# darcamo/pyphysim

Measured on AMD Instinct MI355X. Metric: Monte Carlo realizations/sec (whole node) + SER abs-error vs ref, higher is better.
Workload: dtype f64

## Files before the change

pyphysim_amd/csrc/c4_select.hpp:

```cpp
#pragma once
#include <cstdio>
#include "../../include/mcle.h"

namespace mcle {

enum : int { WDEC_GENERIC = 0, WDEC_SLICER = 1, WDEC_QAM_CERT = 2, WDEC_QUAD_CERT = 3, WDEC_AXIS4_CERT = 4 };

enum : int {
    C4_THR_DEFAULT = 0,
    C4_THR_R4_AH4 = 256,
    C4_THR_R16_ALT = 257,
    C4_THR_R16_TABLE = 258,
    C4_THR_R16_FUSED = 259,
    C4_THR_WAVE = 260,
    C4_THR_PLANAR = 261,
    C4_THR_WAVE_ALT = 262,
    C4_THR_PW4 = 263,
    C4_THR_PW4_W2 = 264,
    C4_THR_PW_TIME = 265,
    C4_THR_PW_CLASS = 266,
    C4_THR_PW_PLANES = 267,
    C4_THR_PW_HALVES = 268,
    C4_THR_512 = 512,
    C4_THR_1024 = 1024,
};
constexpr bool c4_threads_accepted(long long v) {
    return v == C4_THR_DEFAULT || (v >= C4_THR_R4_AH4 && v <= C4_THR_PW_HALVES) || v == C4_THR_512 || v == C4_THR_1024;
}

struct C4Query {
    bool f64;
    int fft_size, nt, nr, num_used, cp_size;
    int M;
    int dec;
    long long f64_threads, f64_generic, no_mfma, f32_mfma, mfma_variant;
#ifdef MCLE_EXPERIMENTS
    long long f64_variant;
#endif
};

enum : int { C4_REFUSED_SHAPE = 0, C4_GENERIC, C4_PLANAR, C4_FW, C4_QW, C4_PW, C4_MFMA };

struct C4Plan {
    int family = C4_REFUSED_SHAPE;
    bool f64 = true;
    int n = 0, nt = 0, nr = 0;
    int ah = 0;
    int wps = 0;
    int variant = 0;
    bool td = false, rows = false, halves = false;
    char asked = 0;
    int abl = 0;
};

#ifndef MCLE_PLANAR_F32_WPS_PLUS
#define MCLE_PLANAR_F32_WPS_PLUS 2
#endif
#ifndef MCLE_PLANAR_F64_256_WPS3
#define MCLE_PLANAR_F64_256_WPS3 0
#endif
constexpr int planar_wps(bool f64, int n, int nt, int nr, int w64) {
    if (!f64 && w64 <= 3 && ((n == 256 && !(nt == 4 && nr == 4)) || (n == 512 && nr == 2))) return w64 + MCLE_PLANAR_F32_WPS_PLUS;
    if (MCLE_PLANAR_F64_256_WPS3 && f64 && n == 256 && nr <= 3 && w64 == 2) return 3;
    return w64;
}

constexpr int planar_r4_ah(int nr) { return nr == 3 ? 3 : 2; }
constexpr int planar_r4_wps(bool f64, int n, int nt, int nr) {
    const int w64 = nr == 3 ? 2 : nr == 2 ? (n == 256 ? 2 : n == 2048 ? 4 : 3) : (n <= 512 ? 3 : 4);
    return planar_wps(f64, n, nt, nr, w64);
}

#ifdef MCLE_EXPERIMENTS
constexpr bool c4_abl_wave(long long v) { return (v >= 32 && v <= 1024 && (v & (v - 1)) == 0) || v == 2016; }
constexpr bool c4_abl_qw(long long v) { return c4_abl_wave(v) || v == 384; }
constexpr bool c4_abl_planar(long long v) { return c4_abl_qw(v) || v == 1920; }
#endif

inline bool c4_select_planar(const C4Query& q, C4Plan& p) {
    const int n = q.fft_size, nt = q.nt, nr = q.nr;
    const long long thr = q.f64_threads;
    if (!(n == 256 || n == 512 || n == 1024 || n == 2048) || nr < 2 || nr > 4 || nt < 1 || nt > nr) return false;
    if (n == 256 && nt == 2 && nr == 2) return false;
    p.family = C4_PLANAR;
    p.ah = planar_r4_ah(nr);
    p.wps = planar_r4_wps(q.f64, n, nt, nr);
    p.variant = 0;
    if (n == 1024 && nr == 4) {
        const int r16_wps = q.f64 ? 2 : 4, r16_var = q.f64 ? 12 : 4;
        if (nt < 4) {
            if (thr == C4_THR_DEFAULT) p.ah = 4, p.wps = r16_wps, p.variant = r16_var;
            return true;
        }
#ifdef MCLE_EXPERIMENTS
        if (q.f64 && q.f64_variant >= 1 && q.f64_variant <= 3) {
            p.variant = (int)q.f64_variant;
            return true;
        }
        if (q.f64 && c4_abl_planar(q.f64_variant)) {
            p.ah = 4, p.wps = 2, p.variant = 12 | (int)q.f64_variant;
            return true;
        }
#endif
        if (thr == C4_THR_512) return true;
        p.ah = 4, p.wps = r16_wps, p.variant = r16_var;
        if (thr == C4_THR_R4_AH4) p.wps = 2, p.variant = 0;
        else if (q.f64 && thr == C4_THR_R16_TABLE) p.variant = 28;
        else if (q.f64 && thr == C4_THR_R16_ALT) p.variant = 4;
        else if (!q.f64 && thr == C4_THR_R16_ALT) p.wps = 3;
        else if (!q.f64 && thr == C4_THR_R16_FUSED) p.variant = 12;
        return true;
    }
    if (n == 2048 && nr == 4 && (thr == C4_THR_512 || (thr != C4_THR_1024 && (nt == 4 || !q.f64)))) p.ah = 4, p.wps = 2;
    return true;
}

inline C4Plan c4_select(const C4Query& q) {
    const int n = q.fft_size, nt = q.nt, nr = q.nr;
    const long long thr = q.f64_threads;
    const bool sq4 = nt == 4 && nr == 4;
    C4Plan p;
    p.f64 = q.f64, p.n = n, p.nt = nt, p.nr = nr;
    if (!q.f64 && q.f32_mfma && !q.no_mfma && n == 1024 && sq4) {
        p.family = C4_MFMA;
        p.variant = q.mfma_variant ? (int)q.mfma_variant : 36;
        return p;
    }
    const bool has_generic = nt == nr && (nt == 2 || nt == 4);
    const bool want_generic = has_generic && (q.f64_generic || (!q.f64 && q.no_mfma));
    if (!want_generic) {
        const bool wave = q.num_used == n && (q.cp_size & 1) == 0 && q.M <= 256 && q.dec != WDEC_GENERIC;
        const bool wave_thr = thr == C4_THR_DEFAULT || thr == C4_THR_WAVE || thr == C4_THR_WAVE_ALT;
        if (wave && n == 256 && has_generic && wave_thr) {
            p.family = C4_FW;
            p.wps = (thr == C4_THR_WAVE_ALT) == q.f64 ? 2 : 3;
#ifdef MCLE_EXPERIMENTS
            if (q.f64 && sq4 && c4_abl_wave(q.f64_variant)) p.wps = 3, p.abl = (int)q.f64_variant;
#endif
            return p;
        }
        const bool pw_thr = thr == C4_THR_DEFAULT || (thr >= C4_THR_PW_TIME && thr <= C4_THR_PW_HALVES) ||
                            (n == 1024 ? thr == C4_THR_PW4 || thr == C4_THR_PW4_W2 : thr == C4_THR_WAVE || thr == C4_THR_WAVE_ALT);
        if (wave && q.f64 && sq4 && (n == 512 || n == 1024 || n == 2048) && pw_thr) {
            p.family = C4_PW;
            p.wps = n == 2048 ? 2 : 3;
            p.td = thr == C4_THR_PW_TIME;
            p.rows = !p.td && thr != C4_THR_PW_CLASS;
            p.halves = p.rows && (thr == C4_THR_PW_HALVES || (thr != C4_THR_PW_PLANES && n != 512));
            p.asked = thr == C4_THR_PW_PLANES ? 'x' : thr == C4_THR_PW_HALVES ? 'h' : 0;
            if (n != 2048) {
                if (thr == C4_THR_WAVE_ALT || thr == C4_THR_PW4_W2) p.wps = 2;
#ifdef MCLE_EXPERIMENTS
                if ((thr < C4_THR_PW_CLASS || thr > C4_THR_PW_HALVES) && c4_abl_wave(q.f64_variant))
                    p.wps = 3, p.halves = false, p.abl = (int)q.f64_variant;
#endif
            }
            return p;
        }
        if (wave && q.f64 && sq4 && n == 1024 && wave_thr && (q.dec == WDEC_SLICER || q.dec == WDEC_QAM_CERT || q.dec == WDEC_QUAD_CERT)) {
            p.family = C4_QW;
            p.wps = thr == C4_THR_WAVE_ALT ? 2 : 3;
#ifdef MCLE_EXPERIMENTS
            if (c4_abl_qw(q.f64_variant)) p.wps = 3, p.abl = (int)q.f64_variant;
#endif
            return p;
        }
        if (c4_select_planar(q, p)) return p;
    }
    if (has_generic) p.family = C4_GENERIC;
    return p;
}

inline void c4_plan_tag(const C4Plan& p, char* out, int len) {
    const char* dt = p.f64 ? "f64" : "f32";
    switch (p.family) {
        case C4_GENERIC: std::snprintf(out, (size_t)len, "mimo_ofdm_generic<%d,%d> %s", p.n, p.nt, dt); break;
        case C4_PLANAR: std::snprintf(out, (size_t)len, "mimo_ofdm_planar<%d,%d,%d> %s ah%d w%d v%d", p.n, p.nt, p.nr, dt, p.ah, p.wps, p.variant); break;
        case C4_FW: std::snprintf(out, (size_t)len, "mimo_ofdm_fw<%d> %s w%d", p.nt, dt, p.wps); break;
        case C4_QW: std::snprintf(out, (size_t)len, "mimo_ofdm_qw w%d", p.wps); break;
        case C4_PW:
            std::snprintf(out, (size_t)len, "mimo_ofdm_pw<%d>/%s%s%s", p.n / 256, p.td ? "time" : "freq", p.wps == (p.n == 2048 ? 2 : 3) ? "" : "/w2",
                          !p.td && !p.rows ? "/a" : p.asked == 'x' ? "/x" : p.asked == 'h' ? "/h" : "");
            break;
        case C4_MFMA: std::snprintf(out, (size_t)len, "mimo_ofdm_mfma v%d", p.variant); break;
        default: if (len > 0) out[0] = 0; break;
    }
}

}
```

pyphysim_amd/csrc/mimo_planar_common.hpp:

```cpp
#pragma once
#include <type_traits>
#include <utility>

#include "fft.hpp"
#include "fft_r16.hpp"
#include "mimo.hpp"
#include "modem.hpp"
#include "philox.hpp"
#include "totals.hpp"
#include "pipe_common.hpp"

namespace mcle {

struct MimoParams {
    int cp, num_used, n_ofdm_sym;
    int mmse;
    double noise_var;
};

template <int NT, int NR> constexpr int d64_rec() { return 2 * NT * NR + 1; }


template <typename T, int N, int NT, int NR>
__global__ __launch_bounds__(64) void k_mimo_filters_planar(MimoParams pp, uint64_t seed, uint64_t first, uint64_t count,
                                                            cx<T>* __restrict__ recs) {
    constexpr int kRec = d64_rec<NT, NR>();
    const uint64_t rl = (uint64_t)blockIdx.x * 64 + threadIdx.x;
    if (rl >= count) return;
    const double rx_scale = sqrt((double)(pp.num_used + pp.cp)) / (double)N;
    const Rng rng(seed, first + rl);
    cx<T>* rec = recs + rl * kRec;
    double2 H[NR][NT], G[NT][NR];
#pragma unroll
    for (int r = 0; r < NR; ++r)
#pragma unroll
        for (int a = 0; a < NT; ++a) {
            const cx<T> h = cn_sample<T>(rng, STREAM_CHAN, (uint64_t)(r * NT + a), (T)1);
            rec[r * NT + a] = h;
            H[r][a] = mk<double>((double)h.x, (double)h.y);
        }
    const bool ok = blast_filter<NT, NR>(H, pp.mmse ? pp.noise_var : 0.0, G);
#pragma unroll
    for (int a = 0; a < NT; ++a)
#pragma unroll
        for (int r = 0; r < NR; ++r) rec[NT * NR + a * NR + r] = mk<T>((T)(G[a][r].x * rx_scale), (T)(G[a][r].y * rx_scale));
    rec[2 * NT * NR] = mk<T>(ok ? (T)0 : (T)1, (T)0);
}

template <typename T, int N, int NT, int NR, typename Link>
inline int launch_sliced_planar(mcle_ctx* ctx, const MimoParams& pp, uint64_t seed, uint64_t first, uint64_t count, uint64_t k_slice,
                                uint32_t* d_sym, uint32_t* d_bit, Link&& link) {
    return launch_sliced(ctx, first, count, k_slice, d64_rec<NT, NR>() * sizeof(cx<T>), d_sym, d_bit,
                         [&](void* recs, uint64_t at, uint64_t n) {
                             hipLaunchKernelGGL((k_mimo_filters_planar<T, N, NT, NR>), dim3((unsigned)((n + 63) / 64)), dim3(64), 0,
                                                ctx->stream, pp, seed, at, n, (cx<T>*)recs);
                         },
                         link);
}

__device__ __forceinline__ void swap32_pair(double a, double b, double& x, double& y) {
    const auto lo = __builtin_amdgcn_permlane32_swap((unsigned)__double2loint(a), (unsigned)__double2loint(b), false, false);
    const auto hi = __builtin_amdgcn_permlane32_swap((unsigned)__double2hiint(a), (unsigned)__double2hiint(b), false, false);
    x = __hiloint2double((int)hi[0], (int)lo[0]);
    y = __hiloint2double((int)hi[1], (int)lo[1]);
}
__device__ __forceinline__ void swap32_pair(float a, float b, float& x, float& y) {
    const auto v = __builtin_amdgcn_permlane32_swap(__float_as_uint(a), __float_as_uint(b), false, false);
    x = __uint_as_float(v[0]);
    y = __uint_as_float(v[1]);
}

__device__ __forceinline__ double2 cn_words(uint32_t x0, uint32_t x1, double sigma, const double* s_bm) {
    return cn_from_words_lds(x0, x1, sigma, s_bm);
}
__device__ __forceinline__ float2 cn_words(uint32_t x0, uint32_t x1, float sigma, const double*) { return cn_from_words(x0, x1, sigma); }

}
```

pyphysim_amd/csrc/pipeline_mimo_pw.hip:

```cpp
#include "mimo_planar_common.hpp"
#include "walk_f64.hpp"

namespace mcle {

constexpr int kPwPlane = 4 * 272;
__host__ __device__ __forceinline__ int pw_slot(int a, int e) { return a * 272 + e + (e >> 4); }
__host__ __device__ __forceinline__ int pw_mtime(int h, int c) { return (c & 3) * 64 + (c >> 2) * 16 + (h & 3) * 4 + (h >> 2); }
template <int NW> constexpr int pw_lab_stride() { return 16 * NW + 16; }
template <int NW> constexpr size_t pw_static_lds() {
    return (size_t)((kBmLdsDoubles + 1) & ~1) * sizeof(double) + (size_t)64 * pw_lab_stride<NW>() + 2 * (d64_rec<4, 4>() + 1) * sizeof(double2) +
           64 * sizeof(unsigned) + sizeof(WgTotals);
}

__device__ __forceinline__ void pw_row_swap(uint32_t& x, uint32_t& y) {
#if defined(__HIP_DEVICE_COMPILE__)
#if __has_builtin(__builtin_amdgcn_permlane16_swap)
    const auto s = __builtin_amdgcn_permlane16_swap(x, y, false, false);
    x = s[0];
    y = s[1];
#else
    const bool odd = (__lane_id() & 16) != 0;
    const uint32_t give = odd ? x : y, got = (uint32_t)__shfl_xor((int)give, 16);
    if (odd) x = got;
    else y = got;
#endif
#endif
}

template <int NW, int J, bool STUB>
__device__ __forceinline__ void pw_first_stage(const unsigned char* lab_row, const double2* s_txtab, const double2* __restrict__ g_tw,
                                               double2 (&v)[16]) {
    const uint4* lab = reinterpret_cast<const uint4*>(lab_row);
    if constexpr (NW == 4) {
#pragma unroll
        for (int i = 0; i < 4; ++i) {
            const uint4 L = lab[i];
            const uint32_t wds[4] = {L.x, L.y, L.z, L.w};
#pragma unroll
            for (int uu = 0; uu < 4; ++uu) {
                const int u = 4 * i + uu;
                const uint32_t w = wds[uu];
                double2 X0, X1, X2, X3;
                if constexpr (STUB) {
                    X0 = X1 = X2 = X3 = mk<double>((double)w, 1.0);
                } else {
                    X0 = s_txtab[w & 0xFFu];
                    X1 = s_txtab[(w >> 8) & 0xFFu];
                    X2 = s_txtab[(w >> 16) & 0xFFu];
                    X3 = s_txtab[w >> 24];
                }
                const double2 A = (J & 1) ? csub(X0, X2) : cadd(X0, X2);
                const double2 B = (J & 1) ? csub(X1, X3) : cadd(X1, X3);
                double2 S;
                if constexpr (J == 0) S = cadd(A, B);
                else if constexpr (J == 1) S = mk<double>(A.x - B.y, A.y + B.x);
                else if constexpr (J == 2) S = csub(A, B);
                else S = mk<double>(A.x + B.y, A.y - B.x);
                if constexpr (J == 0) v[u] = S;
                else if (u == 0) v[u] = S;
                else v[u] = cmulc(S, g_tw[16 * J * u]);
            }
        }
    } else if constexpr (NW == 8) {
        constexpr double kH = 0.70710678118654752440;
// ... 16 lines not shown
#pragma unroll
                    for (int q = 0; q < 8; ++q) X[q] = mk<double>((double)(w0 + w1), 1.0);
                } else {
#pragma unroll
                    for (int q = 0; q < 4; ++q) {
                        X[q] = s_txtab[(w0 >> (8 * q)) & 0xFFu];
                        X[q + 4] = s_txtab[(w1 >> (8 * q)) & 0xFFu];
                    }
                }
                double2 A[4];
#pragma unroll
                for (int q = 0; q < 4; ++q) A[q] = (J & 1) ? csub(X[q], X[q + 4]) : cadd(X[q], X[q + 4]);
                const double2 B0 = cadd(A[0], rotJ(A[2])), B1 = cadd(A[1], rotJ(A[3]));
                double2 S;
                if constexpr (J == 0) S = cadd(B0, B1);
                else if constexpr (J == 2) S = mk<double>(B0.x - B1.y, B0.y + B1.x);
                else if constexpr (J == 4) S = csub(B0, B1);
                else if constexpr (J == 6) S = mk<double>(B0.x + B1.y, B0.y - B1.x);
                else {
                    constexpr double c = (J == 1 || J == 7) ? kH : -kH, sn = (J == 1 || J == 3) ? kH : -kH;
                    S = mk<double>(B0.x + (c * B1.x - sn * B1.y), B0.y + (sn * B1.x + c * B1.y));
                }
                if constexpr (J == 0) v[u] = S;
                else if (u == 0) v[u] = S;
                else v[u] = cmulc(S, g_tw[16 * J * u]);
            }
        }
    } else {
        static_assert(NW == 2, "first stage");
#pragma unroll
        for (int i = 0; i < 2; ++i) {
            const uint4 L = lab[i];
            const uint32_t wds[4] = {L.x, L.y, L.z, L.w};
#pragma unroll
            for (int uu = 0; uu < 8; ++uu) {
                const int u = 8 * i + uu;
                const uint32_t w = wds[uu >> 1] >> (16 * (uu & 1));
                double2 X0, X1;
                if constexpr (STUB) {
                    X0 = X1 = mk<double>((double)(w & 0xFFFFu), 1.0);
                } else {
                    X0 = s_txtab[w & 0xFFu];
                    X1 = s_txtab[(w >> 8) & 0xFFu];
                }
                const double2 S = J ? csub(X0, X1) : cadd(X0, X1);
                if constexpr (J == 0) v[u] = S;
                else if (u == 0) v[u] = S;
                else v[u] = cmulc(S, g_tw[16 * J * u]);
            }
        }
    }
}

template <int NW, int DEC, int WPS, bool TD = false, int ABL = 0, bool ROWS = !TD, bool XCH = ROWS && !TD>
__global__ __launch_bounds__(64 * NW, WPS) void k_run_mimo_ofdm_pw(MimoParams pp, ModemParams<double> mp, uint64_t seed, uint64_t first,
                                                                   uint64_t count, const double2* __restrict__ g_tw,
                                                                   const double2* __restrict__ g_recs, mcle_counters* counters,
                                                                   uint32_t* __restrict__ sym_out, uint32_t* __restrict__ bit_out) {
    using T = double;
    constexpr int N = 256 * NW, NT = 4, NR = 4, kRec = d64_rec<NT, NR>(), TB = 64 * NW, UU = 16 / NW;
    constexpr int kLabStride = pw_lab_stride<NW>();
    static_assert(NW == 2 || NW == 4 || NW == 8, "wavefronts per realization");
    static_assert(!(TD && ROWS), "the time-domain form keeps the map wavefront = class");
    static_assert(!XCH || (ROWS && ABL == 0), "the exchange in complex halves belongs to the default form by lane row");
    constexpr bool kAhead = ROWS && ABL == 0;
#ifdef MCLE_PW_LATE_B5
    constexpr bool kLateB5 = XCH && kAhead;
#else
    constexpr bool kLateB5 = false;
#endif
    constexpr int kLogNW = NW == 2 ? 1 : NW == 4 ? 2 : 3;
    extern __shared__ __attribute__((aligned(16))) char pw_smem[];
    constexpr int kBm = (kBmLdsDoubles + 1) & ~1;
    __shared__ __attribute__((aligned(16))) double s_bm[kBm];
    __shared__ __attribute__((aligned(16))) unsigned char s_lab[64 * kLabStride];
    __shared__ __attribute__((aligned(16))) cx<T> s_rec[2 * (kRec + 1)];
    __shared__ unsigned s_part[64];
    __shared__ WgTotals totals;
    static_assert(sizeof(s_bm) + sizeof(s_lab) + sizeof(s_rec) + sizeof(s_part) + sizeof(totals) == pw_static_lds<NW>(), "launcher's LDS sum");
    T* s_R = reinterpret_cast<T*>(pw_smem);
    cx<T>* s_table = reinterpret_cast<cx<T>*>(s_R + NW * kPwPlane);
    cx<T>* s_txtab = s_table + ((mp.M + 1) & ~1);

    const int tid = threadIdx.x, lane = tid & 63;
    const int j = __builtin_amdgcn_readfirstlane(tid >> 6);
    const int pj = j & 1;
    const int cp = pp.cp;
    const int per_sym = N * NT;
    const uint64_t row = (uint64_t)pp.n_ofdm_sym * (N + cp);
    const T sigma = (T)sqrt(pp.noise_var);
    const T tx_scale = (T)(1.0 / sqrt((double)NT) / sqrt((double)(N + cp)));
    const T tab_scale = TD ? tx_scale : tx_scale * (T)N;
    const uint32_t mask = (uint32_t)(mp.M - 1);
    for (int m = tid; m < mp.M; m += TB) {
        const cx<T> c = mp.g_table[m];
        s_table[m] = c;
        s_txtab[m] = cscale(c, tab_scale);
    }
    if constexpr (ROWS) bm_tables_to_lds_pairs(s_bm, tid, TB);
    else bm_tables_to_lds(s_bm, tid, TB);
    if (tid == 0) wg_zero(totals);

    T* s_mine = s_R + j * kPwPlane;
    uint2* s_words_mine = reinterpret_cast<uint2*>(s_mine);
    using Pass = std::conditional_t<kAhead, uint32_t, uint64_t>;
    Pass it = 0;
    uint64_t rl_prev = 0;
    cx<T> rec_next = mk<T>(0, 0);
    if (tid < kRec && blockIdx.x < count) rec_next = g_recs[(uint64_t)blockIdx.x * kRec + tid];
    unsigned step = 0;
    if constexpr (kAhead) {
        step = gridDim.x;
        asm volatile("" : "+s"(step));
    }
    auto grid_step = [&]() -> unsigned {
        if constexpr (kAhead) return step;
        else return gridDim.x;
    };
    __syncthreads();
    for (uint64_t rl = blockIdx.x; rl < count; rl += grid_step(), ++it) {
        const Rng rng(seed, first + rl);
        const int buf = (int)(it & 1);
        if (tid < kRec) {
            s_rec[buf * (kRec + 1) + tid] = rec_next;
            if (rl + grid_step() < count) rec_next = g_recs[(rl + grid_step()) * kRec + tid];
        }
        const cx<T>* s_H = s_rec + buf * (kRec + 1);
        const cx<T>* s_G = s_H + NT * NR;
        unsigned se = 0, be = 0;
        for (int os = 0; os < pp.n_ofdm_sym; ++os) {
            if constexpr (!kLateB5) {
                if (it > 0 || os > 0) __syncthreads();
            }
            if constexpr (ROWS && !(ABL & 128)) __builtin_amdgcn_s_waitcnt(0xC07F);
            {
                const int t = opaque(tid);
                Words4 dw;
                if constexpr (ABL & 32) dw.w[0] = dw.w[1] = dw.w[2] = dw.w[3] = (uint32_t)t * 0x01010101u;
                else dw = rng.block(STREAM_DATA, (uint32_t)(((uint64_t)os * per_sym) >> 4) + (uint32_t)t);
                const int q = (t >> 6) ^ (NW / 2), u = (t & 63) >> 2;
#pragma unroll
                for (int s = 0; s < 4; ++s) {
                    const uint32_t w = dw.w[s] & (mask * 0x01010101u);
                    const int g = 4 * (t & 3) + s;
                    unsigned char* dst = s_lab + g * kLabStride + NW * u + q;
#pragma unroll
                    for (int a = 0; a < 4; ++a) dst[a * 16 * kLabStride] = (unsigned char)(w >> (8 * a));
                }
            }
            if constexpr (!ROWS) {
                const int ln = opaque(lane);
                const int r = ln >> 4, h = ln & 15;
                const uint64_t i00 = (uint64_t)r * row + (uint64_t)os * (N + cp) + cp + (j & ~1) + 32 * NW * pj + NW * (uint64_t)pw_mtime(h, 0);
                const uint32_t b0 = (uint32_t)(i00 >> 1);
                uint2* w_even = reinterpret_cast<uint2*>(s_R + (j & ~1) * kPwPlane) + (8 * pj) * 64 + ln;
                uint2* w_odd = reinterpret_cast<uint2*>(s_R + (j | 1) * kPwPlane) + (8 * pj) * 64 + ln;
#pragma unroll
                for (int cc = 0; cc < 8; ++cc) {
                    Words4 b;
                    if constexpr (ABL & 128) b.w[0] = b.w[1] = b.w[2] = b.w[3] = b0 + cc;
                    else b = rng.block(STREAM_NOISE, b0 + (uint32_t)(NW / 2) * (uint32_t)pw_mtime(0, cc));
                    w_even[cc * 64] = make_uint2(b.w[0], b.w[1]);
                    w_odd[cc * 64] = make_uint2(b.w[2], b.w[3]);
                }
            }
            auto account_prev = [&]() {
                if (tid == 0 && os == 0 && it > 0) {
                    const unsigned* qq = s_part + (buf ^ 1) * 32;
                    unsigned ts = 0, tb = 0;
#pragma unroll
                    for (int i = 0; i < NW; ++i) {
                        ts += qq[2 * i];
                        tb += qq[2 * i + 1];
                    }
                    uint64_t rp = rl_prev;
                    if constexpr (kAhead) {
                        uint64_t here = rl;
                        asm volatile("" : "+s"(here));
                        rp = here - step;
                    }
                    wg_account(totals, ts, tb, s_rec[(buf ^ 1) * (kRec + 1) + 2 * NT * NR].x != 0.0, rp, sym_out, bit_out);
                }
            };
            if constexpr (!ROWS) {
                __syncthreads();
                account_prev();
            }
            cx<T> v[16];
            if constexpr (TD) {
                const int ln = opaque(lane);
                const unsigned char* lab = s_lab + ln * kLabStride;
                if constexpr (NW == 4) {
                    switch (j) {
                        case 0: pw_first_stage<4, 0, (ABL & 32) != 0>(lab, s_txtab, g_tw, v); break;
                        case 1: pw_first_stage<4, 1, (ABL & 32) != 0>(lab, s_txtab, g_tw, v); break;
                        case 2: pw_first_stage<4, 2, (ABL & 32) != 0>(lab, s_txtab, g_tw, v); break;
                        default: pw_first_stage<4, 3, (ABL & 32) != 0>(lab, s_txtab, g_tw, v); break;
                    }
                } else if constexpr (NW == 8) {
                    switch (j) {
                        case 0: pw_first_stage<8, 0, (ABL & 32) != 0>(lab, s_txtab, g_tw, v); break;
                        case 1: pw_first_stage<8, 1, (ABL & 32) != 0>(lab, s_txtab, g_tw, v); break;
                        case 2: pw_first_stage<8, 2, (ABL & 32) != 0>(lab, s_txtab, g_tw, v); break;
                        case 3: pw_first_stage<8, 3, (ABL & 32) != 0>(lab, s_txtab, g_tw, v); break;
                        case 4: pw_first_stage<8, 4, (ABL & 32) != 0>(lab, s_txtab, g_tw, v); break;
                        case 5: pw_first_stage<8, 5, (ABL & 32) != 0>(lab, s_txtab, g_tw, v); break;
                        case 6: pw_first_stage<8, 6, (ABL & 32) != 0>(lab, s_txtab, g_tw, v); break;
                        default: pw_first_stage<8, 7, (ABL & 32) != 0>(lab, s_txtab, g_tw, v); break;
                    }
                } else {
                    if (j == 0) pw_first_stage<2, 0, (ABL & 32) != 0>(lab, s_txtab, g_tw, v);
                    else pw_first_stage<2, 1, (ABL & 32) != 0>(lab, s_txtab, g_tw, v);
                }
            }
            if constexpr (TD && !(ABL & 64)) {
                const int g = opaque(lane) & 15;
                R16Tw64<T> tw;
#pragma unroll
                for (int m = 1; m <= 3; ++m) {
                    tw.a1[m - 1] = g_tw[g * (NW * m + j)];
                    tw.a2[m - 1] = g_tw[4 * NW * g * m];
                }
                const cx<T> f0 = g_tw[g * j];
                r16_pass<T, true, false, 0, false, true, true>(nullptr, nullptr, 0, tw, nullptr, 0, v, v);
#pragma unroll
                for (int q = 0; q < 4; ++q) v[q] = cmulc(v[q], f0);
            }
            uint2 nw[16];
            if constexpr (!ROWS) {
                const int ln = opaque(lane);
#pragma unroll
                for (int c = 0; c < 16; ++c) nw[c] = s_words_mine[c * 64 + ln];
            }
            if constexpr (TD) {
                const int ln = opaque(lane);
                const int a = ln >> 4, g = ln & 15;
// ... 98 lines not shown
                const int wbase = pw_slot(a, g), rbase = pw_slot(a, 16 * g);
                T xr[16];
                if constexpr (kLateB5) {
#pragma unroll
                    for (int c = 0; c < 16; ++c) asm volatile("" : "+v"(v[c].x), "+v"(v[c].y));
                    if (it > 0 || os > 0) __syncthreads();
                }
#pragma unroll
                for (int c = 0; c < 16; ++c) s_mine[rbase + c] = v[c].x;
                walk_wave_order();
#pragma unroll
                for (int u = 0; u < 16; ++u) xr[u] = s_mine[wbase + 17 * u];
                walk_wave_order();
#pragma unroll
                for (int c = 0; c < 16; ++c) s_mine[rbase + c] = v[c].y;
                walk_wave_order();
#pragma unroll
                for (int u = 0; u < 16; ++u) v[u] = mk<T>(xr[u], s_mine[wbase + 17 * u]);
            }
            if constexpr (!(ABL & 512)) {
                if constexpr (!kAhead) {
                    const int g = opaque(lane) & 15;
#pragma unroll
                    for (int m = 1; m <= 3; ++m) {
                        tw1.a1[m - 1] = g_tw[NW * g * m];
                        tw1.a2[m - 1] = g_tw[4 * NW * g * m];
                    }
                }
                r16_pass<T, false, true, 0, false, true, true>(nullptr, nullptr, 0, tw1, nullptr, 0, v, v);
            }
            T er[NW][UU], ei[NW][UU];
            cx<T> ez[NW][UU];
            constexpr uint32_t kTwBytes = (uint32_t)sizeof(cx<T>);
            uint32_t kp0 = 0;
            static_assert(16 * kTwBytes * (NW - 1) * (UU - 1) < 4096, "the load's immediate offset");
            auto tw_at = [&](int m, int uu) {
                const char* lane_base = reinterpret_cast<const char*>(g_tw) + (size_t)(kTwBytes * (uint32_t)m * kp0);
                return *reinterpret_cast<const cx<T>*>(lane_base + 16 * (int)kTwBytes * m * uu);
            };
            cx<T> twb[2][NW - 1];
            uint4 lab_ahead = make_uint4(0, 0, 0, 0);
            cx<T> hA_ahead = mk<T>(0, 0), gA_ahead = mk<T>(0, 0);
            if constexpr (XCH) {
                const int ln = opaque(lane);
                const int r = ln >> 4, g = ln & 15;
                constexpr int UH = UU / 2, kSl = 272 / 2;
                cx<T>* s_X = reinterpret_cast<cx<T>*>(s_R);
                const int wA = (4 * j + r) * kSl + g;
                const int rA = NW * r * kSl + g + 16 * UH * j;
                const int rB = NW == 2 ? (4 * (r & 1) + j) * kSl + g + 16 * UH * (r >> 1) : j * kSl + g + 16 * UH * (NW / 4) * r;
                r16_wave_sync();
#pragma unroll
                for (int u = 0; u < 16; ++u) asm volatile("" : "+v"(v[u].x));
                account_prev();
#pragma unroll
                for (int u = 0; u < 16; ++u) asm volatile("" : "+v"(v[u].y));
#pragma unroll
                for (int jw = 0; jw < NW; ++jw)
#pragma unroll
                    for (int uu = 0; uu < UH; ++uu) s_X[wA + 16 * (UH * jw + uu)] = v[UU * jw + uu];
                __syncthreads();
#pragma unroll
                for (int jj = 0; jj < NW; ++jj)
#pragma unroll
                    for (int uu = 0; uu < UH; ++uu) ez[jj][uu] = s_X[rA + jj * kSl + 16 * uu];
#pragma unroll
                for (int jw = 0; jw < NW; ++jw)
#pragma unroll
                    for (int uu = UH; uu < UU; ++uu) s_X[rA + jw * kSl + 16 * (uu - UH)] = v[UU * jw + uu];
                kp0 = (uint32_t)opaque((ln & 15) + 16 * UU * j);
#pragma unroll
                for (int m = 1; m < NW; ++m) twb[0][m - 1] = tw_at(m, 0);
                lab_ahead = *reinterpret_cast<const uint4*>(s_lab + ln * kLabStride + 16 * j);
                hA_ahead = s_H[(ln & 3) * NT + (ln >> 4)];
                gA_ahead = s_G[(ln & 3) * NR + (ln >> 4)];
                __syncthreads();
#pragma unroll
                for (int jj = 0; jj < NW; ++jj) {
                    const int off = NW == 2 ? 2 * jj * kSl : (jj & 3) * NW * kSl + 16 * UH * (jj >> 2);
#pragma unroll
                    for (int uu = UH; uu < UU; ++uu) ez[jj][uu] = s_X[rB + off + 16 * (uu - UH)];
                }
            } else {
                const int ln = opaque(lane);
                const int r = ln >> 4, g = ln & 15;
                constexpr int kClass = ROWS ? 272 : kPwPlane;
                const int wpos = r * 272 + g + (ROWS ? 16 * (((4 * j + r) >> kLogNW) & 1) : 0);
                const int rpos = (ROWS ? NW * r * 272 + 16 * (r & 1) : r * 272) + g + 16 * UU * j;
                r16_wave_sync();
#pragma unroll
                for (int u = 0; u < 16; ++u) s_mine[wpos + 16 * u] = v[u].x;
                __syncthreads();
                if constexpr (ROWS) account_prev();
#pragma unroll
                for (int jj = 0; jj < NW; ++jj)
#pragma unroll
                    for (int uu = 0; uu < UU; ++uu) er[jj][uu] = s_R[jj * kClass + rpos + 16 * uu];
                __syncthreads();
#pragma unroll
                for (int u = 0; u < 16; ++u) s_mine[wpos + 16 * u] = v[u].y;
                if constexpr (kAhead) {
                    kp0 = (uint32_t)opaque((ln & 15) + 16 * UU * j);
#pragma unroll
                    for (int m = 1; m < NW; ++m) twb[0][m - 1] = tw_at(m, 0);
                    lab_ahead = *reinterpret_cast<const uint4*>(s_lab + ln * kLabStride + 16 * j);
                    hA_ahead = s_H[(ln & 3) * NT + (ln >> 4)];
                    gA_ahead = s_G[(ln & 3) * NR + (ln >> 4)];
                }
                __syncthreads();
#pragma unroll
                for (int jj = 0; jj < NW; ++jj)
#pragma unroll
                    for (int uu = 0; uu < UU; ++uu) ei[jj][uu] = s_R[jj * kClass + rpos + 16 * uu];
            }
            if constexpr (!(ABL & 1024)) {
                const int ln = opaque(lane);
                if constexpr (!kAhead) kp0 = (uint32_t)opaque((ln & 15) + 16 * UU * j);
                auto ex = [&](int jj, int uu) {
                    if constexpr (XCH) return ez[jj][uu];
                    else return mk<T>(er[jj][uu], ei[jj][uu]);
                };
                auto tw_of = [&](int m, int uu) {
                    if constexpr (kAhead) return twb[uu & 1][m - 1];
                    else return tw_at(m, uu);
                };
#pragma unroll
                for (int uu = 0; uu < UU; ++uu) {
                    if constexpr (kAhead) {
                        if (uu + 1 < UU) {
#pragma unroll
                            for (int m = 1; m < NW; ++m) twb[(uu + 1) & 1][m - 1] = tw_at(m, uu + 1);
                        }
                        __builtin_amdgcn_sched_barrier(0);
                    }
                    if constexpr (NW == 4) {
                        const cx<T> w1 = tw_of(1, uu), w2 = tw_of(2, uu), w3 = tw_of(3, uu);
                        const cx<T> u0 = ex(0, uu);
                        const cx<T> u1 = cmul(ex(1, uu), w1);
                        const cx<T> u2 = cmul(ex(2, uu), w2);
                        const cx<T> u3 = cmul(ex(3, uu), w3);
                        CxOps<T>::template bfly4<false>(u0, u1, u2, u3, v[4 * uu], v[4 * uu + 1], v[4 * uu + 2], v[4 * uu + 3]);
                    } else if constexpr (NW == 8) {
                        cx<T> x[8];
                        x[0] = ex(0, uu);
#pragma unroll
                        for (int jj = 1; jj < 8; ++jj) x[jj] = cmul(ex(jj, uu), tw_of(jj, uu));
// ... 44 lines not shown
                            yi[jj] = __builtin_amdgcn_mfma_f64_4x4x4f64(him, X[jj].x, v[4 * i + jj].y, 0, 0, 0);
                        }
#pragma unroll
                        for (int jj = 0; jj < 4; ++jj) {
                            yr[jj] = __builtin_amdgcn_mfma_f64_4x4x4f64(nhim, X[jj].y, yr[jj], 0, 0, 0);
                            yi[jj] = __builtin_amdgcn_mfma_f64_4x4x4f64(hre, X[jj].y, yi[jj], 0, 0, 0);
                            v[4 * i + jj] = mk<T>(yr[jj], yi[jj]);
                        }
                    }
                }
                if constexpr (!(ABL & 1024)) {
                cx<T> gA;
                if constexpr (kAhead) gA = gA_ahead;
                else gA = s_G[(ln & 3) * NR + (ln >> 4)];
                const T gre = gA.x, gim = gA.y, ngim = -gA.y;
#pragma unroll
                for (int i = 0; i < 4; ++i) {
                    cx<T> e[4];
#pragma unroll
                    for (int jj = 0; jj < 4; ++jj) {
                        const int u = 4 * i + jj;
                        T xr = __builtin_amdgcn_mfma_f64_4x4x4f64(gre, v[u].x, 0.0, 0, 0, 0);
                        T xi = __builtin_amdgcn_mfma_f64_4x4x4f64(gim, v[u].x, 0.0, 0, 0, 0);
                        xr = __builtin_amdgcn_mfma_f64_4x4x4f64(ngim, v[u].y, xr, 0, 0, 0);
                        xi = __builtin_amdgcn_mfma_f64_4x4x4f64(gre, v[u].y, xi, 0, 0, 0);
                        e[jj] = mk<T>(xr, xi);
                    }
                    if constexpr (DEC == WDEC_SLICER || DEC == WDEC_QAM_CERT) {
                        walk_qam_count4<DEC == WDEC_QAM_CERT>(mp, s_table, e, wds[i], se, be);
                    } else {
                        int tx[4];
#pragma unroll
                        for (int jj = 0; jj < 4; ++jj) tx[jj] = (int)((wds[i] >> (8 * jj)) & 0xFFu);
                        walk_decide<DEC, 4>(mp, s_table, nullptr, e, tx, se, be);
                    }
                }
                } else {
                    T keep = er[0][0] + ei[NW - 1][UU - 1];
                    if constexpr (!TD) {
#pragma unroll
                        for (int u = 0; u < 16; ++u) keep += v[u].x + v[u].y;
                    }
                    se += (unsigned)(keep == 0.5) + (wds[0] == 0x12345u);
                }
            }
        }
        if constexpr (kAhead) {
            se = walk_wave_total(se);
            be = walk_wave_total(be);
        } else {
            se = wave_sum_u32(se);
            be = wave_sum_u32(be);
        }
        if (lane == 0) {
            s_part[buf * 32 + 2 * j] = se;
            s_part[buf * 32 + 2 * j + 1] = be;
        }
        rl_prev = rl;
    }
    __syncthreads();
    if (tid == 0) {
        if (it > 0) {
            const int buf = (int)((it - 1) & 1);
            const unsigned* qq = s_part + buf * 32;
            unsigned ts = 0, tb = 0;
#pragma unroll
            for (int i = 0; i < NW; ++i) {
                ts += qq[2 * i];
                tb += qq[2 * i + 1];
            }
            if constexpr (kAhead) rl_prev = blockIdx.x + (uint64_t)(it - 1) * step;
            wg_account(totals, ts, tb, s_rec[buf * (kRec + 1) + 2 * NT * NR].x != 0.0, rl_prev, sym_out, bit_out);
        }
        wg_flush(totals, counters, (unsigned long long)per_sym * pp.n_ofdm_sym, (unsigned long long)per_sym * pp.n_ofdm_sym * mp.bits);
    }
}

template <int NW, int WPS, bool TD, int ABL, bool ROWS, bool XCH>
static int launch_mimo_ofdm_pw(mcle_ctx* ctx, const C4Plan& plan, const mcle_mimo_ofdm_cfg* cfg, uint64_t seed, uint64_t first,
                               uint64_t count, mcle_counters* d_counters, uint32_t* d_sym, uint32_t* d_bit) {
    using T = double;
    constexpr int N = 256 * NW, NT = 4, NR = 4;
    int rc;
    void* tw = nullptr;
    if ((rc = ctx->get_twiddles(N, MCLE_F64, &tw))) return rc;
    MimoParams pp{cfg->cp_size, cfg->num_used, cfg->n_ofdm_sym, cfg->mmse, cfg->noise_var};
    ModemParams<T> mp = pipe_modem<T>(ctx, cfg->demod_method);
    const int dec = walk_dec_kind(ctx, mp);
    mp.grid.G = 0;
    const size_t tab_len = ((size_t)mp.M + 1) & ~(size_t)1;
    const size_t dyn = (size_t)NW * kPwPlane * sizeof(T) + 2 * tab_len * sizeof(cx<T>);
    const size_t lds = dyn + pw_static_lds<NW>();
    MCLE_REQUIRE(lds + 512 <= (size_t)160 * 1024, "part-wave MIMO-OFDM kernel: %zu B of LDS do not fit", lds);
    auto kern = k_run_mimo_ofdm_pw<NW, WDEC_SLICER, WPS, TD, ABL, ROWS, XCH>;
    switch (dec) {
        case WDEC_QAM_CERT: kern = k_run_mimo_ofdm_pw<NW, WDEC_QAM_CERT, WPS, TD, ABL, ROWS, XCH>; break;
        case WDEC_QUAD_CERT: kern = k_run_mimo_ofdm_pw<NW, WDEC_QUAD_CERT, WPS, TD, ABL, ROWS, XCH>; break;
        case WDEC_AXIS4_CERT: kern = k_run_mimo_ofdm_pw<NW, WDEC_AXIS4_CERT, WPS, TD, ABL, ROWS, XCH>; break;
        default: break;
    }
    MCLE_HIP(hipFuncSetAttribute((const void*)kern, hipFuncAttributeMaxDynamicSharedMemorySize, (int)dyn));
    int per_cu = (int)((size_t)160 * 1024 / (lds + 512));
    if (per_cu < 1) per_cu = 1;
    const int by_waves = WPS * 4 / NW;
    if (per_cu > by_waves) per_cu = by_waves;
    const uint64_t resident = (uint64_t)ctx->n_cu * per_cu;
    static_assert(XCH ? ROWS && ABL == 0 : true, "the exchange in complex halves: default form by lane row only");
    set_c4_kernel(ctx, plan);
    const uint64_t kSlice = 1ull << 20;
    return launch_sliced_planar<T, N, NT, NR>(ctx, pp, seed, first, count, kSlice, d_sym, d_bit,
                                              [&](void* recs, uint64_t at, uint64_t n, uint32_t* sym, uint32_t* bit) {
        const unsigned grid = (unsigned)oversubscribed_grid(ctx, resident, n, 8, NW == 4 ? 32 : 16);
        hipLaunchKernelGGL(kern, dim3(grid), dim3(64 * NW), dyn, ctx->stream, pp, mp, seed, at, n, (const cx<T>*)tw, (const cx<T>*)recs,
                           d_counters, sym, bit);
    });
}

int launch_mimo_ofdm_pw(mcle_ctx* ctx, const C4Plan& p, const mcle_mimo_ofdm_cfg* cfg, uint64_t seed, uint64_t first, uint64_t count,
                        mcle_counters* d_counters, uint32_t* d_sym, uint32_t* d_bit) {
#define MCLE_PW(NW_, WPS_, TD_, ABL_, ROWS_, XCH_)                                                                              \
    if (p.n == 256 * NW_ && p.wps == WPS_ && p.td == TD_ && p.abl == ABL_ && p.rows == ROWS_ && p.halves == XCH_)               \
        return launch_mimo_ofdm_pw<NW_, WPS_, TD_, ABL_, ROWS_, XCH_>(ctx, p, cfg, seed, first, count, d_counters, d_sym, d_bit);
#define MCLE_PW_SIZE(NW_, WPS_)                                                                                                 \
    MCLE_PW(NW_, WPS_, false, 0, false, false) MCLE_PW(NW_, WPS_, false, 0, true, true) MCLE_PW(NW_, WPS_, false, 0, true, false) \
    MCLE_PW(NW_, WPS_, true, 0, false, false)
    MCLE_PW_SIZE(2, 3) MCLE_PW(2, 2, false, 0, true, false)
    MCLE_PW_SIZE(4, 3) MCLE_PW(4, 2, false, 0, true, true)
    MCLE_PW_SIZE(8, 2)
#ifdef MCLE_EXPERIMENTS
#define MCLE_PW_ABL(V_)                                                                                                         \
    MCLE_PW(2, 3, true, V_, false, false) MCLE_PW(2, 3, false, V_, true, false) MCLE_PW(4, 3, true, V_, false, false)           \
    MCLE_PW(4, 3, false, V_, true, false)
    MCLE_PW_ABL(32) MCLE_PW_ABL(64) MCLE_PW_ABL(128) MCLE_PW_ABL(256) MCLE_PW_ABL(512) MCLE_PW_ABL(1024) MCLE_PW_ABL(2016)
#undef MCLE_PW_ABL
#endif
#undef MCLE_PW_SIZE
#undef MCLE_PW
    MCLE_REQUIRE(false, "internal: no part-wave MIMO-OFDM kernel <%d> w%d time %d rows %d halves %d ablation %d", p.n / 256, p.wps, (int)p.td,
                 (int)p.rows, (int)p.halves, p.abl);
}

}
```

Baseline: 50.41 million.

## Move part-wave per-realization error accounting into a separate fold kernel

```diff
diff --git a/pyphysim_amd/csrc/c4_select.hpp b/pyphysim_amd/csrc/c4_select.hpp
--- a/pyphysim_amd/csrc/c4_select.hpp
+++ b/pyphysim_amd/csrc/c4_select.hpp
@@ -21,11 +21,13 @@
     C4_THR_PW_CLASS = 266,
     C4_THR_PW_PLANES = 267,
     C4_THR_PW_HALVES = 268,
+    C4_THR_PW_INLOOP = 269,
+    C4_THR_PW_FOLD = 270,
     C4_THR_512 = 512,
     C4_THR_1024 = 1024,
 };
 constexpr bool c4_threads_accepted(long long v) {
-    return v == C4_THR_DEFAULT || (v >= C4_THR_R4_AH4 && v <= C4_THR_PW_HALVES) || v == C4_THR_512 || v == C4_THR_1024;
+    return v == C4_THR_DEFAULT || (v >= C4_THR_R4_AH4 && v <= C4_THR_PW_FOLD) || v == C4_THR_512 || v == C4_THR_1024;
 }
 
 struct C4Query {
@@ -50,6 +52,7 @@
     int variant = 0;
     bool td = false, rows = false, halves = false;
     char asked = 0;
+    bool fold = false;
     int abl = 0;
 };
 
@@ -70,6 +73,8 @@
     const int w64 = nr == 3 ? 2 : nr == 2 ? (n == 256 ? 2 : n == 2048 ? 4 : 3) : (n <= 512 ? 3 : 4);
     return planar_wps(f64, n, nt, nr, w64);
 }
+
+constexpr bool c4_pw_fold_default(int n) { return n == 512 || n == 2048; }
 
 #ifdef MCLE_EXPERIMENTS
 constexpr bool c4_abl_wave(long long v) { return (v >= 32 && v <= 1024 && (v & (v - 1)) == 0) || v == 2016; }
@@ -139,7 +144,7 @@
 #endif
             return p;
         }
-        const bool pw_thr = thr == C4_THR_DEFAULT || (thr >= C4_THR_PW_TIME && thr <= C4_THR_PW_HALVES) ||
+        const bool pw_thr = thr == C4_THR_DEFAULT || (thr >= C4_THR_PW_TIME && thr <= C4_THR_PW_FOLD) ||
                             (n == 1024 ? thr == C4_THR_PW4 || thr == C4_THR_PW4_W2 : thr == C4_THR_WAVE || thr == C4_THR_WAVE_ALT);
         if (wave && q.f64 && sq4 && (n == 512 || n == 1024 || n == 2048) && pw_thr) {
             p.family = C4_PW;
@@ -147,14 +152,15 @@
             p.td = thr == C4_THR_PW_TIME;
             p.rows = !p.td && thr != C4_THR_PW_CLASS;
             p.halves = p.rows && (thr == C4_THR_PW_HALVES || (thr != C4_THR_PW_PLANES && n != 512));
-            p.asked = thr == C4_THR_PW_PLANES ? 'x' : thr == C4_THR_PW_HALVES ? 'h' : 0;
+            p.asked = thr == C4_THR_PW_PLANES ? 'x' : thr == C4_THR_PW_HALVES ? 'h' : thr == C4_THR_PW_INLOOP ? 'k' : thr == C4_THR_PW_FOLD ? 'f' : 0;
             if (n != 2048) {
                 if (thr == C4_THR_WAVE_ALT || thr == C4_THR_PW4_W2) p.wps = 2;
 #ifdef MCLE_EXPERIMENTS
-                if ((thr < C4_THR_PW_CLASS || thr > C4_THR_PW_HALVES) && c4_abl_wave(q.f64_variant))
+                if ((thr < C4_THR_PW_CLASS || thr > C4_THR_PW_FOLD) && c4_abl_wave(q.f64_variant))
                     p.wps = 3, p.halves = false, p.abl = (int)q.f64_variant;
 #endif
             }
+            p.fold = p.rows && p.abl == 0 && p.wps == (n == 2048 ? 2 : 3) && (p.asked == 'f' || (p.asked == 0 && c4_pw_fold_default(n)));
             return p;
         }
         if (wave && q.f64 && sq4 && n == 1024 && wave_thr && (q.dec == WDEC_SLICER || q.dec == WDEC_QAM_CERT || q.dec == WDEC_QUAD_CERT)) {
@@ -180,7 +186,7 @@
         case C4_QW: std::snprintf(out, (size_t)len, "mimo_ofdm_qw w%d", p.wps); break;
         case C4_PW:
             std::snprintf(out, (size_t)len, "mimo_ofdm_pw<%d>/%s%s%s", p.n / 256, p.td ? "time" : "freq", p.wps == (p.n == 2048 ? 2 : 3) ? "" : "/w2",
-                          !p.td && !p.rows ? "/a" : p.asked == 'x' ? "/x" : p.asked == 'h' ? "/h" : "");
+                          !p.td && !p.rows ? "/a" : p.asked == 'x' ? "/x" : p.asked == 'h' ? "/h" : p.asked == 'k' ? "/k" : p.asked == 'f' ? "/f" : "");
             break;
         case C4_MFMA: std::snprintf(out, (size_t)len, "mimo_ofdm_mfma v%d", p.variant); break;
         default: if (len > 0) out[0] = 0; break;
diff --git a/pyphysim_amd/csrc/fold_counts.hpp b/pyphysim_amd/csrc/fold_counts.hpp
--- /dev/null
+++ b/pyphysim_amd/csrc/fold_counts.hpp
@@ -0,0 +1,74 @@
+#pragma once
+#include "totals.hpp"
+
+namespace mcle {
+
+constexpr int kFoldThreads = 1024;
+
+template <int NW>
+__global__ __launch_bounds__(kFoldThreads) void k_fold_counts(const uint2* __restrict__ part, const double2* __restrict__ recs,
+                                                              int rec_stride, int flag_at, uint64_t n, mcle_counters* counters,
+                                                              uint32_t* __restrict__ sym_out, uint32_t* __restrict__ bit_out,
+                                                              unsigned long long n_sym, unsigned long long n_bits) {
+    static_assert(NW == 2 || NW == 4 || NW == 8, "pairs per realization: 16-byte reads");
+    __shared__ unsigned long long s_tot[kFoldThreads / 64][6];
+    const int tid = threadIdx.x, lane = tid & 63, wave = tid >> 6;
+    unsigned long long t[6] = {0ull, 0ull, 0ull, 0ull, 0ull, 0ull};
+    const uint64_t stride = (uint64_t)gridDim.x * kFoldThreads;
+    for (uint64_t rl = (uint64_t)blockIdx.x * kFoldThreads + tid; rl < n; rl += stride) {
+        const uint4* q = reinterpret_cast<const uint4*>(part + rl * NW);
+        unsigned se = 0, be = 0;
+#pragma unroll
+        for (int i = 0; i < NW / 2; ++i) {
+            const uint4 w = q[i];
+            se += w.x + w.z;
+            be += w.y + w.w;
+        }
+        const bool skipped = recs[rl * (uint64_t)rec_stride + (uint64_t)flag_at].x != 0.0;
+        if (sym_out) sym_out[rl] = skipped ? 0xFFFFFFFFu : se;
+        if (bit_out) bit_out[rl] = skipped ? 0xFFFFFFFFu : be;
+        if (skipped) {
+            ++t[5];
+        } else {
+            ++t[4];
+            t[0] += se;
+            t[1] += (unsigned long long)se * se;
+            t[2] += be;
+            t[3] += (unsigned long long)be * be;
+        }
+    }
+#pragma unroll
+    for (int k = 0; k < 6; ++k) {
+#pragma unroll
+        for (int d = 32; d >= 1; d >>= 1) t[k] += __shfl_down(t[k], d, 64);
+        if (lane == 0) s_tot[wave][k] = t[k];
+    }
+    __syncthreads();
+    if (tid != 0) return;
+    WgTotals w;
+    wg_zero(w);
+#pragma unroll 1
+    for (int i = 0; i < kFoldThreads / 64; ++i) {
+        w.se += s_tot[i][0];
+        w.se2 += s_tot[i][1];
+        w.be += s_tot[i][2];
+        w.be2 += s_tot[i][3];
+        w.ok += s_tot[i][4];
+        w.skip += s_tot[i][5];
+    }
+    wg_flush(w, counters, n_sym, n_bits);
+}
+
+template <int NW>
+inline void launch_fold_counts(hipStream_t stream, int max_wgs, const uint2* part, const double2* recs, int rec_stride, int flag_at,
+                               uint64_t n, mcle_counters* counters, uint32_t* sym_out, uint32_t* bit_out, unsigned long long n_sym,
+                               unsigned long long n_bits) {
+    if (n == 0) return;
+    uint64_t grid = (n + kFoldThreads - 1) / kFoldThreads;
+    if (max_wgs < 1) max_wgs = 1;
+    if (grid > (uint64_t)max_wgs) grid = (uint64_t)max_wgs;
+    hipLaunchKernelGGL((k_fold_counts<NW>), dim3((unsigned)grid), dim3(kFoldThreads), 0, stream, part, recs, rec_stride, flag_at, n,
+                       counters, sym_out, bit_out, n_sym, n_bits);
+}
+
+}
diff --git a/pyphysim_amd/csrc/mimo_planar_common.hpp b/pyphysim_amd/csrc/mimo_planar_common.hpp
--- a/pyphysim_amd/csrc/mimo_planar_common.hpp
+++ b/pyphysim_amd/csrc/mimo_planar_common.hpp
@@ -49,13 +49,13 @@
 
 template <typename T, int N, int NT, int NR, typename Link>
 inline int launch_sliced_planar(mcle_ctx* ctx, const MimoParams& pp, uint64_t seed, uint64_t first, uint64_t count, uint64_t k_slice,
-                                uint32_t* d_sym, uint32_t* d_bit, Link&& link) {
+                                uint32_t* d_sym, uint32_t* d_bit, Link&& link, size_t tail_bytes = 0) {
     return launch_sliced(ctx, first, count, k_slice, d64_rec<NT, NR>() * sizeof(cx<T>), d_sym, d_bit,
                          [&](void* recs, uint64_t at, uint64_t n) {
                              hipLaunchKernelGGL((k_mimo_filters_planar<T, N, NT, NR>), dim3((unsigned)((n + 63) / 64)), dim3(64), 0,
                                                 ctx->stream, pp, seed, at, n, (cx<T>*)recs);
                          },
-                         link);
+                         link, tail_bytes);
 }
 
 __device__ __forceinline__ void swap32_pair(double a, double b, double& x, double& y) {
diff --git a/pyphysim_amd/csrc/pipeline_mimo_pw.hip b/pyphysim_amd/csrc/pipeline_mimo_pw.hip
--- a/pyphysim_amd/csrc/pipeline_mimo_pw.hip
+++ b/pyphysim_amd/csrc/pipeline_mimo_pw.hip
@@ -1,5 +1,6 @@
 #include "mimo_planar_common.hpp"
 #include "walk_f64.hpp"
+#include "fold_counts.hpp"
 
 namespace mcle {
 
@@ -7,9 +8,9 @@
 __host__ __device__ __forceinline__ int pw_slot(int a, int e) { return a * 272 + e + (e >> 4); }
 __host__ __device__ __forceinline__ int pw_mtime(int h, int c) { return (c & 3) * 64 + (c >> 2) * 16 + (h & 3) * 4 + (h >> 2); }
 template <int NW> constexpr int pw_lab_stride() { return 16 * NW + 16; }
-template <int NW> constexpr size_t pw_static_lds() {
+template <int NW, bool FOLD = false> constexpr size_t pw_static_lds() {
     return (size_t)((kBmLdsDoubles + 1) & ~1) * sizeof(double) + (size_t)64 * pw_lab_stride<NW>() + 2 * (d64_rec<4, 4>() + 1) * sizeof(double2) +
-           64 * sizeof(unsigned) + sizeof(WgTotals);
+           (FOLD ? 0 : 64 * sizeof(unsigned) + sizeof(WgTotals));
 }
 
 __device__ __forceinline__ void pw_row_swap(uint32_t& x, uint32_t& y) {
@@ -132,11 +133,12 @@
     }
 }
 
-template <int NW, int DEC, int WPS, bool TD = false, int ABL = 0, bool ROWS = !TD, bool XCH = ROWS && !TD>
+template <int NW, int DEC, int WPS, bool TD = false, int ABL = 0, bool ROWS = !TD, bool XCH = ROWS && !TD, bool FOLD = false>
 __global__ __launch_bounds__(64 * NW, WPS) void k_run_mimo_ofdm_pw(MimoParams pp, ModemParams<double> mp, uint64_t seed, uint64_t first,
                                                                    uint64_t count, const double2* __restrict__ g_tw,
                                                                    const double2* __restrict__ g_recs, mcle_counters* counters,
-                                                                   uint32_t* __restrict__ sym_out, uint32_t* __restrict__ bit_out) {
+                                                                   uint32_t* __restrict__ sym_out, uint32_t* __restrict__ bit_out,
+                                                                   uint2* __restrict__ part) {
     using T = double;
     constexpr int N = 256 * NW, NT = 4, NR = 4, kRec = d64_rec<NT, NR>(), TB = 64 * NW, UU = 16 / NW;
     constexpr int kLabStride = pw_lab_stride<NW>();
@@ -144,6 +146,7 @@
     static_assert(!(TD && ROWS), "the time-domain form keeps the map wavefront = class");
     static_assert(!XCH || (ROWS && ABL == 0), "the exchange in complex halves belongs to the default form by lane row");
     constexpr bool kAhead = ROWS && ABL == 0;
+    static_assert(!FOLD || kAhead, "the accounting leaves the loop of the default form by lane row only");
 #ifdef MCLE_PW_LATE_B5
     constexpr bool kLateB5 = XCH && kAhead;
 #else
@@ -155,9 +158,10 @@
     __shared__ __attribute__((aligned(16))) double s_bm[kBm];
     __shared__ __attribute__((aligned(16))) unsigned char s_lab[64 * kLabStride];
     __shared__ __attribute__((aligned(16))) cx<T> s_rec[2 * (kRec + 1)];
-    __shared__ unsigned s_part[64];
+    __shared__ unsigned s_part[FOLD ? 1 : 64];
     __shared__ WgTotals totals;
-    static_assert(sizeof(s_bm) + sizeof(s_lab) + sizeof(s_rec) + sizeof(s_part) + sizeof(totals) == pw_static_lds<NW>(), "launcher's LDS sum");
+    static_assert(sizeof(s_bm) + sizeof(s_lab) + sizeof(s_rec) + (FOLD ? 0 : sizeof(s_part) + sizeof(totals)) == pw_static_lds<NW, FOLD>(),
+                  "launcher's LDS sum");
     T* s_R = reinterpret_cast<T*>(pw_smem);
     cx<T>* s_table = reinterpret_cast<cx<T>*>(s_R + NW * kPwPlane);
     cx<T>* s_txtab = s_table + ((mp.M + 1) & ~1);
@@ -179,7 +183,9 @@
     }
     if constexpr (ROWS) bm_tables_to_lds_pairs(s_bm, tid, TB);
     else bm_tables_to_lds(s_bm, tid, TB);
-    if (tid == 0) wg_zero(totals);
+    if constexpr (!FOLD) {
+        if (tid == 0) wg_zero(totals);
+    }
 
     T* s_mine = s_R + j * kPwPlane;
     uint2* s_words_mine = reinterpret_cast<uint2*>(s_mine);
@@ -262,6 +268,9 @@
                     wg_account(totals, ts, tb, s_rec[(buf ^ 1) * (kRec + 1) + 2 * NT * NR].x != 0.0, rp, sym_out, bit_out);
                 }
             };
+            auto block_boundary = [&]() {
+                if (os == 0) asm volatile("");
+            };
             if constexpr (!ROWS) {
                 __syncthreads();
                 account_prev();
@@ -466,7 +475,8 @@
                 r16_wave_sync();
 #pragma unroll
                 for (int u = 0; u < 16; ++u) asm volatile("" : "+v"(v[u].x));
-                account_prev();
+                if constexpr (FOLD) block_boundary();
+                else account_prev();
 #pragma unroll
                 for (int u = 0; u < 16; ++u) asm volatile("" : "+v"(v[u].y));
 #pragma unroll
@@ -505,7 +515,8 @@
 #pragma unroll
                 for (int u = 0; u < 16; ++u) s_mine[wpos + 16 * u] = v[u].x;
                 __syncthreads();
-                if constexpr (ROWS) account_prev();
+                if constexpr (FOLD) block_boundary();
+                else if constexpr (ROWS) account_prev();
 #pragma unroll
                 for (int jj = 0; jj < NW; ++jj)
 #pragma unroll
@@ -656,12 +667,17 @@
             se = wave_sum_u32(se);
             be = wave_sum_u32(be);
         }
-        if (lane == 0) {
-            s_part[buf * 32 + 2 * j] = se;
-            s_part[buf * 32 + 2 * j + 1] = be;
+        if constexpr (FOLD) {
+            if (lane == 0) part[rl * NW + j] = make_uint2(se, be);
+        } else {
+            if (lane == 0) {
+                s_part[buf * 32 + 2 * j] = se;
+                s_part[buf * 32 + 2 * j + 1] = be;
+            }
+            rl_prev = rl;
         }
-        rl_prev = rl;
     }
+    if constexpr (FOLD) return;
     __syncthreads();
     if (tid == 0) {
         if (it > 0) {
@@ -680,7 +696,7 @@
     }
 }
 
-template <int NW, int WPS, bool TD, int ABL, bool ROWS, bool XCH>
+template <int NW, int WPS, bool TD, int ABL, bool ROWS, bool XCH, bool FOLD>
 static int launch_mimo_ofdm_pw(mcle_ctx* ctx, const C4Plan& plan, const mcle_mimo_ofdm_cfg* cfg, uint64_t seed, uint64_t first,
                                uint64_t count, mcle_counters* d_counters, uint32_t* d_sym, uint32_t* d_bit) {
     using T = double;
@@ -694,13 +710,13 @@
     mp.grid.G = 0;
     const size_t tab_len = ((size_t)mp.M + 1) & ~(size_t)1;
     const size_t dyn = (size_t)NW * kPwPlane * sizeof(T) + 2 * tab_len * sizeof(cx<T>);
-    const size_t lds = dyn + pw_static_lds<NW>();
+    const size_t lds = dyn + pw_static_lds<NW, FOLD>();
     MCLE_REQUIRE(lds + 512 <= (size_t)160 * 1024, "part-wave MIMO-OFDM kernel: %zu B of LDS do not fit", lds);
-    auto kern = k_run_mimo_ofdm_pw<NW, WDEC_SLICER, WPS, TD, ABL, ROWS, XCH>;
+    auto kern = k_run_mimo_ofdm_pw<NW, WDEC_SLICER, WPS, TD, ABL, ROWS, XCH, FOLD>;
     switch (dec) {
-        case WDEC_QAM_CERT: kern = k_run_mimo_ofdm_pw<NW, WDEC_QAM_CERT, WPS, TD, ABL, ROWS, XCH>; break;
-        case WDEC_QUAD_CERT: kern = k_run_mimo_ofdm_pw<NW, WDEC_QUAD_CERT, WPS, TD, ABL, ROWS, XCH>; break;
-        case WDEC_AXIS4_CERT: kern = k_run_mimo_ofdm_pw<NW, WDEC_AXIS4_CERT, WPS, TD, ABL, ROWS, XCH>; break;
+        case WDEC_QAM_CERT: kern = k_run_mimo_ofdm_pw<NW, WDEC_QAM_CERT, WPS, TD, ABL, ROWS, XCH, FOLD>; break;
+        case WDEC_QUAD_CERT: kern = k_run_mimo_ofdm_pw<NW, WDEC_QUAD_CERT, WPS, TD, ABL, ROWS, XCH, FOLD>; break;
+        case WDEC_AXIS4_CERT: kern = k_run_mimo_ofdm_pw<NW, WDEC_AXIS4_CERT, WPS, TD, ABL, ROWS, XCH, FOLD>; break;
         default: break;
     }
     MCLE_HIP(hipFuncSetAttribute((const void*)kern, hipFuncAttributeMaxDynamicSharedMemorySize, (int)dyn));
@@ -712,25 +728,34 @@
     static_assert(XCH ? ROWS && ABL == 0 : true, "the exchange in complex halves: default form by lane row only");
     set_c4_kernel(ctx, plan);
     const uint64_t kSlice = 1ull << 20;
+    constexpr int kRec = d64_rec<NT, NR>();
+    const uint64_t slice = count < kSlice ? count : kSlice;
+    const unsigned long long per_sym = (unsigned long long)N * NT;
     return launch_sliced_planar<T, N, NT, NR>(ctx, pp, seed, first, count, kSlice, d_sym, d_bit,
                                               [&](void* recs, uint64_t at, uint64_t n, uint32_t* sym, uint32_t* bit) {
         const unsigned grid = (unsigned)oversubscribed_grid(ctx, resident, n, 8, NW == 4 ? 32 : 16);
+        uint2* part = FOLD ? reinterpret_cast<uint2*>(static_cast<char*>(recs) + slice * kRec * sizeof(cx<T>)) : nullptr;
         hipLaunchKernelGGL(kern, dim3(grid), dim3(64 * NW), dyn, ctx->stream, pp, mp, seed, at, n, (const cx<T>*)tw, (const cx<T>*)recs,
-                           d_counters, sym, bit);
-    });
+                           d_counters, sym, bit, part);
+        if constexpr (FOLD)
+            launch_fold_counts<NW>(ctx->stream, ctx->n_cu, part, (const cx<T>*)recs, kRec, 2 * NT * NR, n, d_counters, sym, bit,
+                                   per_sym * pp.n_ofdm_sym, per_sym * pp.n_ofdm_sym * mp.bits);
+    }, FOLD ? (size_t)8 * NW : (size_t)0);
 }
 
 int launch_mimo_ofdm_pw(mcle_ctx* ctx, const C4Plan& p, const mcle_mimo_ofdm_cfg* cfg, uint64_t seed, uint64_t first, uint64_t count,
                         mcle_counters* d_counters, uint32_t* d_sym, uint32_t* d_bit) {
-#define MCLE_PW(NW_, WPS_, TD_, ABL_, ROWS_, XCH_)                                                                              \
-    if (p.n == 256 * NW_ && p.wps == WPS_ && p.td == TD_ && p.abl == ABL_ && p.rows == ROWS_ && p.halves == XCH_)               \
-        return launch_mimo_ofdm_pw<NW_, WPS_, TD_, ABL_, ROWS_, XCH_>(ctx, p, cfg, seed, first, count, d_counters, d_sym, d_bit);
+#define MCLE_PW_F(NW_, WPS_, TD_, ABL_, ROWS_, XCH_, FOLD_)                                                                     \
+    if (p.n == 256 * NW_ && p.wps == WPS_ && p.td == TD_ && p.abl == ABL_ && p.rows == ROWS_ && p.halves == XCH_ && p.fold == FOLD_) \
+        return launch_mimo_ofdm_pw<NW_, WPS_, TD_, ABL_, ROWS_, XCH_, FOLD_>(ctx, p, cfg, seed, first, count, d_counters, d_sym, d_bit);
+#define MCLE_PW(NW_, WPS_, TD_, ABL_, ROWS_, XCH_) MCLE_PW_F(NW_, WPS_, TD_, ABL_, ROWS_, XCH_, false)
 #define MCLE_PW_SIZE(NW_, WPS_)                                                                                                 \
     MCLE_PW(NW_, WPS_, false, 0, false, false) MCLE_PW(NW_, WPS_, false, 0, true, true) MCLE_PW(NW_, WPS_, false, 0, true, false) \
     MCLE_PW(NW_, WPS_, true, 0, false, false)
     MCLE_PW_SIZE(2, 3) MCLE_PW(2, 2, false, 0, true, false)
     MCLE_PW_SIZE(4, 3) MCLE_PW(4, 2, false, 0, true, true)
     MCLE_PW_SIZE(8, 2)
+    MCLE_PW_F(2, 3, false, 0, true, false, true) MCLE_PW_F(4, 3, false, 0, true, true, true) MCLE_PW_F(8, 2, false, 0, true, true, true)
 #ifdef MCLE_EXPERIMENTS
 #define MCLE_PW_ABL(V_)                                                                                                         \
     MCLE_PW(2, 3, true, V_, false, false) MCLE_PW(2, 3, false, V_, true, false) MCLE_PW(4, 3, true, V_, false, false)           \
@@ -740,8 +765,9 @@
 #endif
 #undef MCLE_PW_SIZE
 #undef MCLE_PW
-    MCLE_REQUIRE(false, "internal: no part-wave MIMO-OFDM kernel <%d> w%d time %d rows %d halves %d ablation %d", p.n / 256, p.wps, (int)p.td,
-                 (int)p.rows, (int)p.halves, p.abl);
+#undef MCLE_PW_F
+    MCLE_REQUIRE(false, "internal: no part-wave MIMO-OFDM kernel <%d> w%d time %d rows %d halves %d fold %d ablation %d", p.n / 256, p.wps,
+                 (int)p.td, (int)p.rows, (int)p.halves, (int)p.fold, p.abl);
 }
 
 }
```

New measurement: 50.45 million (median of 4 runs). About the same (+0.1%).
